# 0xb4lamx/hocuspocus

Measured on AMD Instinct MI355X. Metric: merged update MB/s (bit-exact vs yjs mergeUpdates), higher is better.
Workload: dtype u8; 1 GPU; C2: 10000 docs x 200 single-char Y.Text insert updates per GPU (documents 'c2-<i>', i < 10000, sharded by fnv1a64(name) mod 1), 1-4 uint32 clients, batched Y.mergeUpdates, inputs resident in HBM; docs_per_gpu=10000, docs_total=10000, updates_total=2000000, bytes_in_total=47221584, bytes_out_total=29357349, parallelism=doc-sharded x1

## Files before the change

hocuspocus_amd/csrc/ygm_kernels.hip:

```cpp
#include <hip/hip_runtime.h>
#include <stdint.h>
#include <stdio.h>
#include <stdlib.h>

#include <atomic>

#include "ygm_common.hpp"
#include "ygm_merge_seq.hpp"
#include "ygm_merge_wave.hpp"
#include "ygm_merge_lean.hpp"
#include "ygm_docmeta.hpp"
#include "ygm_doc_walk.hpp"
#include "ygm_merge_big.hpp"
#include "ygm_seqdoc.hpp"
#include "ygm_v1.hpp"

#ifdef YGM_DIAG
__device__ unsigned long long ygm_diag[32];
#define DIAG_T0 unsigned long long _dt = __builtin_amdgcn_s_memtime();
#define DIAG(i) do { if (threadIdx.x == 0) { unsigned long long _n = __builtin_amdgcn_s_memtime(); atomicAdd(&ygm_diag[i], _n - _dt); _dt = _n; } } while (0)
#define DIAGW(i) do { if ((threadIdx.x & 63) == 0) { unsigned long long _n = __builtin_amdgcn_s_memtime(); atomicAdd(&ygm_diag[8 + (i)], _n - _dt); _dt = _n; } } while (0)
__device__ unsigned long long ygm_diag_ts[16384 * 8];
#define DIAGL_T0 if (threadIdx.x == 0) ygm_diag_ts[(blockIdx.x & 16383u) * 8] = __builtin_amdgcn_s_memrealtime();
#define DIAGL(i) do { if (threadIdx.x == 0) ygm_diag_ts[(blockIdx.x & 16383u) * 8 + 1 + (i)] = __builtin_amdgcn_s_memrealtime(); } while (0)
// ... 815 lines not shown
        fb0 = atomicAdd(&meta->fb_count, (unsigned int)__popcll(bm));
        atomicAdd(&meta->fb_upds, (unsigned long long)su);
        atomicAdd(&meta->fb_bytes, (unsigned long long)sb);
      }
      fb0 = (uint32_t)__shfl((int)fb0, (int)lead);
    }
    if (rm) {
      const uint32_t rl = (uint32_t)__builtin_ctzll(rm);
      if (l == rl) r0 = atomicAdd(&meta->route_n, (unsigned int)__popcll(rm));
      r0 = (uint32_t)__shfl((int)r0, (int)rl);
    }
    if (big) {
      fb_list[fb0 + lanes_below(bm)] = d;
      out_off[d] = merge_slot(upd_off[u0], d); out_len[d] = 0; status[d] = ST_FALLBACK;
    } else if (in) rest[r0 + lanes_below(rm)] = d;
  }
}


struct LeanHdr { uint32_t u0, k; uint64_t b0, nbytes; };

YDEV uint32_t lean_du_load(const uint32_t* __restrict__ doc_upd, uint32_t d, uint32_t n_docs) {
  const uint32_t l = threadIdx.x;
  return d < n_docs ? doc_upd[d + (l & 1u)] : 0u;
}
template <int LENS>
YDEV uint64_t lean_bo_load(const uint64_t* __restrict__ upd_off, const uint64_t* __restrict__ doc_off, uint32_t du, uint32_t d,
                           uint32_t n_docs) {
  if (LENS) return d < n_docs ? doc_off[d + (threadIdx.x & 1u)] : 0ull;
  const uint32_t u0 = rdlane(du, 0), u1 = rdlane(du, 1);
  return d < n_docs ? upd_off[(threadIdx.x & 1u) ? u1 : u0] : 0ull;
}
YDEV LeanHdr lean_hdr_of(uint32_t du, uint64_t bo) {
  LeanHdr h;
  h.u0 = rdlane(du, 0); h.k = rdlane(du, 1) - h.u0;
  const uint64_t b0 = ((uint64_t)rdlane((uint32_t)(bo >> 32), 0) << 32) | rdlane((uint32_t)bo, 0);
  const uint64_t b1 = ((uint64_t)rdlane((uint32_t)(bo >> 32), 1) << 32) | rdlane((uint32_t)bo, 1);
  h.b0 = b0; h.nbytes = b1 - b0;
  return h;
}
YDEV bool ln_owns(uint32_t l, int q, uint32_t n) { return l < ((n + (uint32_t)(LN_ROWS - 1 - q)) >> 2); }
template <int WIDE>
YDEV bool lean_stageable(const LeanHdr& h) {
  return h.k >= 2 && h.k < (uint32_t)(WAVE * LN_ROWS) && (h.b0 & 15u) + h.nbytes <= (uint64_t)LnCfg<WIDE>::IN;
}
template <int WIDE, int LENS = 0>
YDEV void lean_prefetch(const uint8_t* __restrict__ arena, const uint64_t* __restrict__ upd_off, const uint16_t* __restrict__ upd_len,
                        const LeanHdr& h, bool go, u32x4 (&v)[(LnCfg<WIDE>::IN + 16 * WAVE - 1) / (16 * WAVE)],
                        uint32_t (&rx)[LN_ROWS + 1]) {
  const uint32_t l = threadIdx.x;
  const uint64_t a0 = go ? (h.b0 & ~15ull) : 0ull;
  const uint32_t last = go ? (uint32_t)(((h.b0 & 15u) + h.nbytes + 15) / 16) - 1u : 0u;
#pragma unroll
  for (int j = 0; j < (LnCfg<WIDE>::IN + 16 * WAVE - 1) / (16 * WAVE); j++) {
    const uint32_t c = l + WAVE * j;
    v[j] = *(const u32x4*)(arena + a0 + 16ull * (c < last ? c : last));
  }
  const uint32_t kk = go ? h.k : 0u;
  const uint32_t l4 = LN_ROWS * lane_opaque();
  if (LENS) {
#pragma unroll
    for (int q = 0; q < LN_ROWS; q++) {
      const uint32_t i = l4 + q;
      rx[q] = upd_len[h.u0 + (i < kk ? i : 0u)];
    }
    return;
  }
  const uint32_t* off32 = (const uint32_t*)upd_off;
#pragma unroll
  for (int q = 0; q <= LN_ROWS; q++) {
    const uint32_t i = l4 + q;
    rx[q] = off32[2ull * (h.u0 + (i <= kk ? i : 0u))];
  }
}

template <int WIDE, int LENS = 0>
#ifndef YGM_LN_OCC
#define YGM_LN_OCC 4
#endif
__global__ __launch_bounds__(WAVE, WIDE ? 3 : YGM_LN_OCC) void k_merge_lean(const uint8_t* __restrict__ arena, const uint64_t* __restrict__ upd_off,
                                                     const uint32_t* __restrict__ doc_upd, uint32_t n_docs, uint32_t flags,
                                                     uint8_t* __restrict__ out, uint64_t* __restrict__ out_off,
                                                     uint64_t* __restrict__ out_len, int32_t* __restrict__ status, DocMeta* meta,
                                                     DocMeta* __restrict__ meta_next, uint32_t* __restrict__ defer_list, uint64_t out_cap,
                                                     const uint32_t* __restrict__ list, uint32_t n_list,
                                                     const uint64_t* __restrict__ doc_off, const uint16_t* __restrict__ upd_len) {
  typedef LnCfg<WIDE> C;
  __shared__ LeanLdsT<WIDE> LS;
  if (meta_next && blockIdx.x == 0) {
    static_assert(sizeof(DocMeta) % 16 == 0, "DocMeta is zeroed in 16-byte pieces");
    const u32x4 z = {0u, 0u, 0u, 0u};
    for (uint32_t i = threadIdx.x; i < sizeof(DocMeta) / 16; i += WAVE) ((u32x4*)meta_next)[i] = z;
  }
  LB8* lin = (LB8*)LS.in;
  LB8* lout = (LB8*)LS.out;
  const uint32_t l = threadIdx.x;
  const uint32_t G = gridDim.x;
  const bool force_seq = (flags & 2u) != 0;
  const uint32_t n_it = WIDE ? n_list : n_docs;
  auto list_at = [&](uint32_t j) -> uint32_t {
    const uint64_t i = (uint64_t)blockIdx.x + (uint64_t)j * G;
    return i < n_it ? (list ? list[i] : (uint32_t)i) : n_docs;
  };
  uint32_t lst0 = 0, lst1 = 0;
  if (WIDE) { lst0 = list_at(l); lst1 = list_at(WAVE + l); }
  uint32_t it = 0;
  auto docof = [&](uint32_t j) -> uint32_t {
    return (uint32_t)__builtin_amdgcn_readfirstlane((int)rdlane((j >> 6) != (it >> 6) ? lst1 : lst0, j & 63u));
  };
#define LN_AHEAD(k) (WIDE ? docof(it + (k)) : d + (k) * G)
  uint32_t d = WIDE ? (n_it > blockIdx.x ? docof(0) : n_docs) : blockIdx.x;
  (void)n_it;
  uint32_t du = lean_du_load(doc_upd, d, n_docs);
  LeanHdr hn = lean_hdr_of(du, lean_bo_load<LENS>(upd_off, doc_off, du, d, n_docs));
  du = lean_du_load(doc_upd, LN_AHEAD(1), n_docs);
  u32x4 v[(C::IN + 16 * WAVE - 1) / (16 * WAVE)];
  uint32_t rx[LN_ROWS + 1];
#pragma unroll
  for (int q = 0; q <= LN_ROWS; q++) rx[q] = 0;
  bool gn = !force_seq && lean_stageable<WIDE>(hn);
  lean_prefetch<WIDE, LENS>(arena, upd_off, upd_len, hn, gn, v, rx);
  uint64_t payload = 0;
  uint64_t dmask = 0;
  uint32_t dit = 0, dch = d;
  auto flush_defer = [&]() {
    if (!dmask) return;
    uint32_t base = 0;
    if (l == 0) base = atomicAdd(WIDE ? &meta->wide_defer : &meta->lean_defer, (uint32_t)__popcll(dmask));
    base = __shfl(base, 0, WAVE);
    if ((dmask >> l) & 1ull) defer_list[base + lanes_below(dmask)] = WIDE ? lst0 : dch + l * G;
    dmask = 0;
  };
  DIAGSW_T0
  for (; WIDE ? (uint64_t)blockIdx.x + (uint64_t)it * G < n_it : d < n_docs; it++) {
    DIAGL_T0
    if (dit == 64) {
      flush_defer(); dit = 0; dch = d;
      if (WIDE) { lst0 = lst1; lst1 = list_at(it + WAVE + l); }
    }
    const LeanHdr h = hn;
    bool go = gn;
    const uint32_t k = h.k;
    const uint64_t b0 = h.b0, nbytes = h.nbytes;
    const uint64_t slot = merge_slot(b0, d), cap = merge_slot_cap(nbytes);
    const uint32_t shift = (uint32_t)(b0 & 15u);
    uint32_t us[LN_ROWS], un[LN_ROWS];
    DIAGSW_WAIT;
    if (go) {
      const uint32_t nch = (uint32_t)((shift + nbytes + 15) / 16);
#pragma unroll
      for (int j = 0; j < (C::IN + 16 * WAVE - 1) / (16 * WAVE); j++) {
        const uint32_t c = l + WAVE * j;
        if (c < nch) *(LB128*)(lin + 16 * c) = v[j];
      }
      if (LENS) {
        uint32_t tot = 0;
#pragma unroll
        for (int q = 0; q < LN_ROWS; q++) {
          un[q] = ln_owns(l, q, k) ? rx[q] : 0u;
          us[q] = tot;
          tot += un[q];
        }
        const uint32_t inc = dpp_incl_add(tot);
        const uint32_t base = shift + inc - tot;
#pragma unroll
        for (int q = 0; q < LN_ROWS; q++) us[q] += base;
        if (lane63(inc) != (uint32_t)nbytes) go = false;
      } else {
#pragma unroll
        for (int q = 0; q < LN_ROWS; q++) { us[q] = shift + (rx[q] - (uint32_t)b0); un[q] = rx[q + 1] - rx[q]; }
      }
      if (!WIDE) {
        bool lng = false;
#pragma unroll
        for (int q = 0; q < LN_ROWS; q++) lng |= ln_owns(l, q, k) && un[q] > (uint32_t)LN_UMAX;
        if (__ballot(lng)) go = false;
      }
    }
    __builtin_amdgcn_s_waitcnt(0x0F70);
    wave_sync();
    DIAGL(0);
#if defined(YGM_LEAN_STOP) && YGM_LEAN_STOP == 1
    { hn = lean_hdr_of(du, lean_bo_load<LENS>(upd_off, doc_off, du, LN_AHEAD(1), n_docs)); du = lean_du_load(doc_upd, LN_AHEAD(2), n_docs);
      gn = !force_seq && lean_stageable<WIDE>(hn); lean_prefetch<WIDE, LENS>(arena, upd_off, upd_len, hn, gn, v, rx); wave_sync(); dit++; d = LN_AHEAD(1); continue; }
#endif
    const uint64_t bo_next = lean_bo_load<LENS>(upd_off, doc_off, du, LN_AHEAD(1), n_docs);
    const uint32_t du_next = lean_du_load(doc_upd, LN_AHEAD(2), n_docs);
    const bool single = k < 2 && !force_seq;
    bool defer = !go && !single;
    uint32_t size = 0;
    if (single) {
      size = k == 0 ? 2u : (uint32_t)nbytes;
      if (k == 1 && nbytes > 0xFFFFFFFFull) size = 0;
      uint8_t* o = out + slot;
      const bool badlen = upd_len != nullptr && k == 1 && (uint64_t)upd_len[h.u0] != nbytes;
      uint64_t olen = k == 0 ? 2 : nbytes;
      int32_t ost = ST_OK;
      if (badlen) { size = 0; olen = 0; ost = ST_MALFORMED; }
      else if (slot + olen > out_cap) { size = 0; olen = 0; ost = ST_NOMEM; }
      else {
        if (k == 0) { if (l == 0) { o[0] = 0; o[1] = 0; } }
        else for (uint64_t c = lane_opaque(); c * 16 < nbytes; c += WAVE) {
          uint4 x; __builtin_memcpy(&x, arena + b0 + 16 * c, 16);
          *(uint4*)(o + 16 * c) = x;
        }
        payload += olen;
      }
      if (l == 0) { out_off[d] = slot; out_len[d] = olen; status[d] = ost; }
      __builtin_amdgcn_s_waitcnt(0x0F70);
    }
    LRec rec[LN_ROWS];
    bool hs[LN_ROWS], hasd[LN_ROWS];
    bool bad = false;
    bool allfast = false;
#pragma unroll
    for (int q = 0; q < LN_ROWS; q++) { hs[q] = false; hasd[q] = false; }
    if (go && !WIDE && YGM_LN_FASTPARSE) {
      allfast = true;
#pragma unroll
      for (int q = 0; q < LN_ROWS; q++) {
        const bool valid = ln_owns(l, q, k);
        us[q] = valid ? us[q] : shift; un[q] = valid ? un[q] : 0u;
      }
      bool slow[LN_ROWS];
#pragma unroll
      for (int g = 0; g < LN_ROWS; g += YGM_LN_FASTGROUP) {
        LFastIn F[YGM_LN_FASTGROUP];
#pragma unroll
        for (int q = g; q < g + YGM_LN_FASTGROUP; q++) lean_fast_load(lin, us[q], un[q], F[q - g]);
#pragma unroll
        for (int q = g; q < g + YGM_LN_FASTGROUP; q++) {
          const bool valid = ln_owns(l, q, k);
          bool hd;
          const bool fast = q == 0 ? lean_parse_fast<true>(F[q - g], us[q], un[q], valid, rec[q], hd)
                                   : lean_parse_fast<false>(F[q - g], us[q], un[q], valid, rec[q], hd);
          slow[q] = !fast && valid;
          hs[q] = valid && (rec[q].span & 0xFF00u) != 0u;
          hasd[q] = valid && hd;
        }
      }
#pragma unroll
      for (int q = 0; q < LN_ROWS; q++) {
        if (__ballot(slow[q]) == 0) continue;
        allfast = false;
        const bool valid = ln_owns(l, q, k);
        if (valid) { rec[q] = lean_parse<LN_UMAX>(lin, us[q], un[q]); bad |= !rec[q].ok; }
        hs[q] = valid && (rec[q].span & 0xFF00u) != 0u;
        hasd[q] = valid && rec[q].ok && lin[lean_ds_pos(us[q], rec[q].span)] != 0;
      }
    } else if (go) {
#pragma unroll
      for (int q = 0; q < LN_ROWS; q++) {
        const bool valid = ln_owns(l, q, k);
        if (valid) { rec[q] = lean_parse<WIDE ? LNW_UMAX : LN_UMAX>(lin, us[q], un[q]); bad |= !rec[q].ok; }
        else { rec[q].ok = true; rec[q].client = 0; rec[q].clock = 0; rec[q].clen = 0; rec[q].span = 0; }
        hs[q] = valid && (rec[q].span & 0xFF00u) != 0u;
        hasd[q] = valid && rec[q].ok && lin[lean_ds_pos(us[q], rec[q].span)] != 0;
      }
    }
    DIAGL(1);
#ifdef YGM_LEAN_SB
    __builtin_amdgcn_sched_barrier(0);
#endif
    hn = lean_hdr_of(du, bo_next); du = du_next;
    gn = !force_seq && lean_stageable<WIDE>(hn);
    lean_prefetch<WIDE, LENS>(arena, upd_off, upd_len, hn, gn, v, rx);
    defer = defer || __ballot(bad) != 0;
    if (single) { wave_sync(); dit++; d = LN_AHEAD(1); continue; }
#if defined(YGM_LEAN_STOP) && YGM_LEAN_STOP == 2
    if (l == 0) status[d] = (int)bad; wave_sync(); dit++; d = LN_AHEAD(1); continue;
#endif
    if (!defer) {
      uint32_t blk[LN_ROWS];
#pragma unroll
      for (int q = 0; q < LN_ROWS; q++) blk[q] = hs[q] ? 0xFFu : 0xFEu;
      uint32_t ctl = 0, nC = 0;
      uint32_t fcl = 0, fcb[LN_ROWS];
#pragma unroll
      for (int q = 0; q < LN_ROWS; q++) fcb[q] = 0;
      bool sighted = false;
      if (!WIDE && allfast) {
        uint32_t cid[4] = {0u, 0u, 0u, 0u}, fck[4] = {0u, 0u, 0u, 0u};
        bool more = true;
#pragma unroll
        for (int t = 0; t < 4; t++) {
          const bool u0 = blk[0] == 0xFFu, u1 = blk[1] == 0xFFu, u2 = blk[2] == 0xFFu, u3 = blk[3] == 0xFFu;
          const uint64_t m = __builtin_amdgcn_ballot_w64(u0 || u1 || u2 || u3);
          if (m == 0) { more = false; break; }
          const uint32_t fl = (uint32_t)__builtin_ctzll(m);
          const uint32_t cand = rdlane(u0 ? rec[0].client : u1 ? rec[1].client : u2 ? rec[2].client : rec[3].client, fl);
          const uint32_t fc = rdlane(u0 ? rec[0].clock : u1 ? rec[1].clock : u2 ? rec[2].clock : rec[3].clock, fl);
          cid[t] = cand; fck[t] = fc; nC = (uint32_t)t + 1u;
#pragma unroll
          for (int q = 0; q < LN_ROWS; q++) {
            const bool hit = blk[q] == 0xFFu && rec[q].client == cand;
            blk[q] = hit ? 8u * (uint32_t)t : blk[q];
            fcb[q] = hit ? fc : fcb[q];
          }
        }
        if (more) more = __builtin_amdgcn_ballot_w64(blk[0] == 0xFFu || blk[1] == 0xFFu || blk[2] == 0xFFu || blk[3] == 0xFFu) != 0;
        if (more) {
#pragma unroll
          for (int q = 0; q < LN_ROWS; q++) blk[q] = hs[q] ? 0xFFu : 0xFEu;
          nC = 0;
        } else {
          sighted = true;
          uint32_t tab = 0;
#pragma unroll
          for (int t = 3; t >= 0; t--) {
            uint32_t r = 0;
#pragma unroll
            for (int j = 0; j < 4; j++) if (j != t) r = lean_sadd_gt(r, cid[j], cid[t]);
            tab |= r << (8 * t);
            lean_wrlane2(ctl, cid[t], fcl, fck[t], r);
          }
#pragma unroll
          for (int q = 0; q < LN_ROWS; q++) blk[q] = __builtin_amdgcn_ubfe(tab, blk[q], 8u);
        }
      }
      for (int it = 0; !sighted && it <= LN_CMAX; it++) {
        uint32_t mx = 0; bool any = false;
#pragma unroll
        for (int q = 0; q < LN_ROWS; q++) { const bool un_ = blk[q] == 0xFFu; any |= un_; mx = max(mx, un_ ? rec[q].client : 0u); }
        if (__ballot(any) == 0) break;
        if (nC == (uint32_t)LN_CMAX) { defer = true; break; }
        const uint32_t cand = lane63(dpp_incl_max(mx));
#pragma unroll
        for (int q = 0; q < LN_ROWS; q++) if (blk[q] == 0xFFu && rec[q].client == cand) blk[q] = nC;
        ctl = l == nC ? cand : ctl;
        nC++;
      }
      if (!defer) {
        uint32_t cA = 0, cB = 0;
        uint32_t idx[LN_ROWS];
        {
          uint32_t ea[LN_ROWS], ta = 0;
#pragma unroll
          for (int q = 0; q < LN_ROWS; q++) {
            ea[q] = ta;
            ta += (hs[q] && blk[q] < 4u) ? 1u << (8u * (blk[q] & 3u)) : 0u;
          }
          const uint32_t ia = dpp_incl_add(ta);
          cA = lane63(ia);
#pragma unroll
          for (int q = 0; q < LN_ROWS; q++) idx[q] = ia - ta + ea[q];
          if (nC > 4u) {
            uint32_t eb[LN_ROWS], tb = 0;
#pragma unroll
            for (int q = 0; q < LN_ROWS; q++) {
              eb[q] = tb;
              tb += (hs[q] && blk[q] >= 4u) ? 1u << (8u * (blk[q] & 3u)) : 0u;
            }
            const uint32_t ib = dpp_incl_add(tb);
            cB = lane63(ib);
#pragma unroll
            for (int q = 0; q < LN_ROWS; q++) idx[q] = (hs[q] && blk[q] >= 4u) ? ib - tb + eb[q] : idx[q];
          }
#pragma unroll
          for (int q = 0; q < LN_ROWS; q++) idx[q] = (idx[q] >> (8u * (blk[q] & 3u))) & 0xFFu;
        }
        uint32_t osp[LN_ROWS], oex[LN_ROWS];
        uint32_t carry = 0, hcnt = 0, hfc = 0, hpos = 0, hdr_all = 0, HC0 = 0, HC1 = 0, nrec = 0;
        const bool logp = sighted;
        if (logp) {
#pragma unroll
          for (int q = 0; q < LN_ROWS; q++) bad |= hs[q] && rec[q].clock != fcb[q] + idx[q];
          const uint32_t T01 = lean_byte_prefix<0>(hs, blk, rec, osp);
          uint32_t T23 = 0;
          if (nC > 2u) T23 = lean_byte_prefix<1>(hs, blk, rec, osp);
          const uint32_t B0 = T01 & 0xFFFFu, B1 = T01 >> 16, B2 = T23 & 0xFFFFu, B3 = T23 >> 16;
          uint32_t hlen = 0;
          if (l < nC) {
            hcnt = (cA >> (8u * (l & 3u))) & 0xFFu; hfc = fcl;
            hlen = vlen32(hcnt) + vlen32(ctl) + vlen32(hfc);
          }
          const uint32_t h0 = rdlane(hlen, 0), h1 = rdlane(hlen, 1), h2 = rdlane(hlen, 2), h3 = rdlane(hlen, 3);
          const uint32_t O0 = vlen32(nC) + h0, O1 = O0 + h1 + B0, O2 = O1 + h2 + B1, O3 = O2 + h3 + B2;
          const uint32_t O01 = O0 | (O1 << 16), O23 = O2 | (O3 << 16);
          hdr_all = h0 + h1 + h2 + h3;
          carry = B0 + B1 + B2 + B3;
          hpos = lean_field16((l & 2u) ? O23 : O01, l) - hlen;
#pragma unroll
// ... 2252 lines not shown
```

hocuspocus_amd/csrc/ygm_merge_lean.hpp:

```cpp
#pragma once
#include "ygm_common.hpp"
#include "ygm_merge_wave.hpp"

namespace ygm {

#ifndef YGM_LN_IN
#define YGM_LN_IN 5120
#endif
#ifndef YGM_LN_OUT
#define YGM_LN_OUT 4096
#endif
constexpr int LN_IN = YGM_LN_IN;
constexpr int LN_ROWS = 4;
constexpr int LN_UMAX = 32;
constexpr int LN_CMAX = 8;

constexpr int LN_OUT = YGM_LN_OUT;

constexpr int LNW_IN = 7168;
constexpr int LNW_UMAX = 64;
constexpr int LNW_OUT = 6144;

template <int WIDE> struct LnCfg {
  static constexpr int IN = WIDE ? LNW_IN : LN_IN;
// ... 69 lines not shown
}

YDEV uint32_t lean_ds_pos(uint32_t us, uint32_t span) { return span ? (span >> 16) + (span & 0xFFu) : us + 1u; }

struct LRec {
  uint32_t client, clock, clen;
  uint32_t span;
  bool ok;
};

YDEV uint32_t pext32(uint32_t x, uint32_t y, uint32_t n) {
  x &= n >= 4u ? 0xFFFFFFFFu : ((1u << (8u * n)) - 1u);
  x &= 0x7f7f7f7fu;
  x = ((x >> 1) & 0x3f803f80u) | (x & 0x007f007fu);
  x = ((x >> 2) & 0x0fffc000u) | (x & 0x00003fffu);
  return x | (n >= 5u ? (y & 0x7Fu) << 28 : 0u);
}

YDEV uint32_t bsel(uint32_t m, uint32_t x, uint32_t y) { return (x & m) | (y & ~m); }

template <int W>
YDEV void lean_windowW(LB8* in, uint32_t s, uint32_t (&d)[W / 4]) {
  const LB32* w = (const LB32*)(in + (s & ~3u));
  uint32_t L[W / 4 + 1];
#pragma unroll
  for (int j = 0; j <= W / 4; j++) L[j] = w[j];
#pragma unroll
  for (int j = 0; j < W / 4; j++) d[j] = __builtin_amdgcn_alignbyte(L[j + 1], L[j], s & 3u);
}
YDEV void lean_window(LB8* in, uint32_t s, uint32_t (&d)[8]) { lean_windowW<32>(in, s, d); }
YDEV uint32_t top8(uint32_t lo, uint32_t hi) {
  const uint32_t a = __builtin_amdgcn_udot4(lo & 0x80808080u, 0x08040201u, 0u, false);
  return __builtin_amdgcn_udot4(hi & 0x80808080u, 0x80402010u, a, false) >> 7;
}
template <int W> struct LnMask;
template <> struct LnMask<32> { typedef uint32_t T; };
template <> struct LnMask<64> { typedef uint64_t T; };
template <int W>
YDEV typename LnMask<W>::T lean_hmaskW(const uint32_t (&d)[W / 4]) {
  typename LnMask<W>::T H = 0;
#pragma unroll
  for (int j = 0; j < W / 8; j++) H |= (typename LnMask<W>::T)top8(d[2 * j], d[2 * j + 1]) << (8 * j);
  return H;
}
YDEV uint32_t lean_hmask(const uint32_t (&d)[8]) { return lean_hmaskW<32>(d); }
YDEV uint32_t lnctz(uint32_t x) { return (uint32_t)__builtin_ctz(x | 0x80000000u); }
YDEV uint32_t lnctz(uint64_t x) { return (uint32_t)__builtin_ctzll(x | 0x8000000000000000ull); }

template <int W>
YDEV LRec lean_parse(LB8* in, uint32_t s, uint32_t n) {
  typedef typename LnMask<W>::T M;
  constexpr uint32_t WB = (uint32_t)W, WL = WB - 1u;
  constexpr M ONE = 1, ALL = ~(M)0;
  LRec R; R.ok = false; R.client = 0; R.clock = 0; R.clen = 0; R.span = 0;
  if (n < 2 || n > WB) return R;
  uint32_t d[W / 4];
  lean_windowW<W>(in, s, d);
  if ((d[0] & 0xFFu) == 0u) { R.ok = true; return R; }
  const M H = lean_hmaskW<W>(d);
  M Z = 0;
#pragma unroll
  for (int j = 0; j < W / 8; j++)
    Z |= (M)top8((d[2 * j] - 0x01010101u) & ~d[2 * j], (d[2 * j + 1] - 0x01010101u) & ~d[2 * j + 1]) << (8 * j);
  const M V = n >= WB ? ALL : ((ONE << n) - ONE);
  const M T = ~H & V;
  const M HV = H & V;
  LB8* u = in + s;
  const M h2 = HV & (HV >> 1), h4 = h2 & (h2 >> 2), h7 = h4 & (h4 >> 3);
  M bad = h7 | (Z & (HV << 1) & V);
#define LN_VEND(p, e) ((e) = ((p) < WL ? (p) : WL) + lnctz((M)(T >> ((p) < WL ? (p) : WL))))
#define LN_ASCII(p, L) (bad |= (M)(((n - (p) - (L)) & 0x80000000u) | ((L) & ~WL)) | ((HV >> ((p) < WL ? (p) : WL)) & ((ONE << ((L) & WL)) - ONE)))
  const uint32_t b0 = d[0] & 0xFFu, b1 = (d[0] >> 8) & 0xFFu;
  bad |= (M)((b0 ^ 1u) | ((b1 - 1u) & ~127u) | (n < 4u ? 1u : 0u));
  uint32_t e, p;
  LN_VEND(2u, e);
  const uint32_t cl_n = e - 1u;
  const uint32_t client = pext32(__builtin_amdgcn_alignbyte(d[1], d[0], 2u), (d[1] >> 16) & 0xFFu, cl_n);
  bad |= (M)((cl_n > 5u ? 1u : 0u) | (cl_n == 5u ? ((d[1] >> 16) & 0x70u) : 0u));
  p = e + 1u;
  LN_VEND(p, e);
  const uint32_t ck_n = e - p + 1u;
  const uint64_t U01 = ((uint64_t)d[1] << 32) | d[0], U23 = ((uint64_t)d[3] << 32) | d[2];
  const uint64_t cw = (U01 >> (8u * (p & 7u))) | (p & 7u ? (U23 << (64u - 8u * (p & 7u))) : 0ull);
  const uint32_t clock = pext32((uint32_t)cw, (uint32_t)(cw >> 32) & 0xFFu, ck_n);
  bad |= (M)((ck_n > 5u ? 1u : 0u) | (ck_n == 5u ? ((uint32_t)(cw >> 32) & 0x70u) : 0u));
  p = e + 1u;
  const uint32_t sstart = p;
  uint32_t clen = 0;
  constexpr uint32_t PC = WB + 8u;
  uint32_t st = 0;
  do {
    const uint32_t pc = p < PC ? p : PC;
    const uint32_t info = u[pc];
    p = pc + 1u;
    const uint32_t ref = info & 31u;
    bad |= (M)((info == 10u ? 1u : 0u) | ((ref != 1u && ref != 4u) ? 1u : 0u) | ((info & 0xC0u) && (info & 0x20u) ? 1u : 0u));
    {
      const uint32_t pp = p < WL ? p : WL;
      const M t0 = (T >> pp) | (ONE << WL), t1 = t0 & (t0 - ONE), t2 = t1 & (t1 - ONE), t3 = t2 & (t2 - ONE);
      const uint32_t nsk = ((info >> 6) & 1u) + ((info >> 7) & 1u);
      const uint32_t e2 = pp + lnctz(t1) + 1u;
      const uint32_t e4 = pp + lnctz(t3) + 1u;
      p = nsk == 2u ? e4 : nsk == 1u ? e2 : p;
    }
    if ((info & 0xC0u) == 0u) {
      const uint32_t pi = u[p < PC ? p : PC]; p++;
      if (pi == 1u) {
        const uint32_t Lk = u[p < PC ? p : PC]; p++;
        LN_ASCII(p, Lk); p += Lk & WL;
      } else {
        bad |= (M)pi;
        LN_VEND(p, e); p = e + 1u; LN_VEND(p, e); p = e + 1u;
      }
      if (info & 0x20u) {
        const uint32_t Ls = u[p < PC ? p : PC]; p++;
        LN_ASCII(p, Ls); p += Ls & WL;
      }
    }
    if (ref == 1u) {
      LN_VEND(p, e);
      const uint32_t pp = p < WL ? p : WL;
      const uint32_t x = u[pp] | ((uint32_t)u[pp + 1] << 8) | ((uint32_t)u[pp + 2] << 16) | ((uint32_t)u[pp + 3] << 24);
      const uint32_t v = pext32(x, 0u, e - p + 1u);
      bad |= (M)((v == 0u ? 1u : 0u) | ((e - p) > 2u ? 1u : 0u));
      clen += v;
      p = e + 1u;
    } else {
      const uint32_t Lc = u[p < PC ? p : PC]; p++;
      bad |= (M)(Lc == 0u ? 1u : 0u);
      LN_ASCII(p, Lc);
      p += Lc & WL;
      clen += Lc;
    }
  } while (++st < b1 && (bad | (M)(p >= n ? 1u : 0u)) == 0);
#undef LN_VEND
#undef LN_ASCII
  bad |= (M)((n - 1u - p) & 0x80000000u);
  bad |= (M)(uint32_t)(((uint64_t)clock + clen) >> 32);
  R.ok = bad == 0;
  R.client = client; R.clock = clock; R.clen = clen;
  R.span = ((s + sstart) << 16) | (b1 << 8) | ((p - sstart) & 0xFFu);
  return R;
}

#ifndef YGM_LN_FASTPARSE
#define YGM_LN_FASTPARSE 1
#endif
#ifndef YGM_LN_FASTGROUP
#define YGM_LN_FASTGROUP 4
#endif
#ifndef YGM_LN_FASTPARENT
#define YGM_LN_FASTPARENT 1
#endif
struct LFastIn {
  uint32_t d[8];
  uint32_t tl, td;
};
YDEV void lean_fast_load(LB8* in, uint32_t s, uint32_t n, LFastIn& F) {
  lean_window(in, s, F.d);
  const uint32_t t = s + (n > 3u ? n : 3u);
  F.tl = in[t - 3u]; F.td = in[t - 1u];
}
#ifndef YGM_LN_KEYGATE
#define YGM_LN_KEYGATE 1
#endif
template <bool KEYROW>
YDEV bool lean_parse_fast(const LFastIn& F, uint32_t s, uint32_t n, bool valid, LRec& R, bool& hasd) {
  const uint32_t (&d)[8] = F.d;
  const uint32_t H = lean_hmask(d);
  uint32_t Z = 0;
#pragma unroll
  for (int j = 0; j < 4; j++)
    Z |= top8((d[2 * j] - 0x01010101u) & ~d[2 * j], (d[2 * j + 1] - 0x01010101u) & ~d[2 * j + 1]) << (8 * j);
  const uint32_t V = n >= 32u ? 0xFFFFFFFFu : ((1u << n) - 1u);
  const uint32_t T = ~H & V, HV = H & V;
  const uint32_t h2 = HV & (HV >> 1), h4 = h2 & (h2 >> 2), h7 = h4 & (h4 >> 3);
  uint32_t bad = h7 | (Z & (HV << 1) & V);
  const uint32_t b0 = d[0] & 0xFFu, b1 = (d[0] >> 8) & 0xFFu;
  bad |= (b0 ^ 1u) | (b1 ^ 1u);
  uint32_t e = 2u + lnctz(T >> 2);
  const uint32_t cl_n = e - 1u;
  const uint32_t client = pext32(__builtin_amdgcn_alignbyte(d[1], d[0], 2u), (d[1] >> 16) & 0xFFu, cl_n);
  bad |= (cl_n > 5u ? 1u : 0u) | (cl_n == 5u ? ((d[1] >> 16) & 0x70u) : 0u);
  const uint32_t p = e + 1u;
  const uint32_t pc = p < 31u ? p : 31u;
  e = pc + lnctz(T >> pc);
  const uint32_t ck_n = e - p + 1u;
  const uint64_t U01 = ((uint64_t)d[1] << 32) | d[0], U23 = ((uint64_t)d[3] << 32) | d[2];
  const uint64_t cw = (U01 >> (8u * (p & 7u))) | (p & 7u ? (U23 << (64u - 8u * (p & 7u))) : 0ull);
  const uint32_t clock = pext32((uint32_t)cw, (uint32_t)(cw >> 32) & 0xFFu, ck_n);
  bad |= (ck_n > 5u ? 1u : 0u) | (ck_n == 5u ? ((uint32_t)(cw >> 32) & 0x70u) : 0u);
  bad |= clock == 0xFFFFFFFFu ? 1u : 0u;
  const uint32_t ip = e + 1u;
  const uint32_t x3 = (uint32_t)(cw >> (8u * (ck_n & 7u)));
  const uint32_t info = x3 & 0xFFu;
  const uint32_t nsk = ((info >> 6) & 1u) + ((info >> 7) & 1u);
  const uint32_t pp = ip + 1u < 31u ? ip + 1u : 31u;
  const uint32_t t0 = (T >> pp) | 0x80000000u, t1 = t0 & (t0 - 1u), t2 = t1 & (t1 - 1u), t3 = t2 & (t2 - 1u);
  const uint32_t pl = nsk == 2u ? pp + lnctz(t3) + 1u : pp + lnctz(t1) + 1u;
  bool fits = pl + 3u == n;
  bool shape = nsk != 0u && (info & 0x3Fu) == 4u;
#if YGM_LN_FASTPARENT
  if (KEYROW || !YGM_LN_KEYGATE || __ballot(valid && nsk == 0u) != 0) {
    const uint32_t lk = (x3 >> 16) & 0xFFu;
    const uint32_t kp = ip + 3u < 31u ? ip + 3u : 31u;
    const bool par = x3 << 16 == 0x01040000u && lk < 32u && ((HV >> kp) & ((1u << (lk & 31u)) - 1u)) == 0u;
    fits = nsk == 0u ? ip + 6u + lk == n : fits;
    shape = shape || (nsk == 0u && par);
  }
#endif
  const bool item = bad == 0u && shape && fits && n <= 32u && F.tl == 1u && ((HV >> ((n - 2u) & 31u)) & 1u) == 0u;
  const bool dsonly = b0 == 0u && n >= 2u && n <= 32u;
  R.ok = true;
  R.client = item ? client : 0u; R.clock = item ? clock : 0u; R.clen = item ? 1u : 0u;
  R.span = item ? ((s + ip) << 16) | (1u << 8) | ((n - 1u - ip) & 0xFFu) : 0u;
  hasd = item ? F.td != 0u : b1 != 0u;
  return item || dsonly;
}

YDEV uint32_t w2_byte(const uint32_t (&d)[8], uint32_t p) {
  const uint32_t i = p >> 2;
  const uint32_t m0 = 0u - (i & 1u), m1 = 0u - ((i >> 1) & 1u), m2 = 0u - ((i >> 2) & 1u);
  const uint32_t a0 = bsel(m0, d[1], d[0]), a1 = bsel(m0, d[3], d[2]), a2 = bsel(m0, d[5], d[4]), a3 = bsel(m0, d[7], d[6]);
  const uint32_t b0 = bsel(m1, a1, a0), b1 = bsel(m1, a3, a2);
  return (bsel(m2, b1, b0) >> (8u * (p & 3u))) & 0xFFu;
}
YDEV void w2_vu5(const uint32_t (&d)[8], uint32_t p, uint32_t& x, uint32_t& y) {
  const uint32_t i = p >> 2, s = p & 3u;
  const uint32_t m0 = 0u - (i & 1u), m1 = 0u - ((i >> 1) & 1u);
  const uint32_t lo = bsel(m1, bsel(m0, d[3], d[2]), bsel(m0, d[1], d[0]));
  const uint32_t hi = bsel(m1, bsel(m0, d[4], d[3]), bsel(m0, d[2], d[1]));
  const uint32_t hh = bsel(m1, bsel(m0, d[5], d[4]), bsel(m0, d[3], d[2]));
  x = __builtin_amdgcn_alignbyte(hi, lo, s);
  y = __builtin_amdgcn_alignbyte(hh, hi, s) & 0xFFu;
}

constexpr int LN_DSMAX = 64;
struct LDsCur {
  LB8* u;
  uint32_t T, lim;
  uint32_t p, cl_left, r_left, client, bad;
};
YDEV uint32_t lean_ds_vu(LDsCur& c, uint32_t maxb) {
  const uint32_t pp = c.p < 31u ? c.p : 31u;
  const uint32_t e = pp + (uint32_t)__builtin_ctz((c.T >> pp) | 0x80000000u);
  const uint32_t nb = e - c.p + 1u;
  LB8* b = c.u + pp;
  const uint32_t x = b[0] | ((uint32_t)b[1] << 8) | ((uint32_t)b[2] << 16) | ((uint32_t)b[3] << 24), y = b[4];
  c.bad |= (c.p >= c.lim ? 1u : 0u) | (e >= c.lim ? 1u : 0u) | (nb > maxb ? 1u : 0u) | (nb == 5u ? (y & 0x70u) : 0u);
  c.p = e + 1u;
  return pext32(x, y, nb);
}
YDEV void lean_ds_open(LB8* in, uint32_t a, uint32_t n, LDsCur& c) {
  uint32_t d[8];
  lean_window(in, a, d);
  c.u = in + a;
  c.lim = n < 32u ? n : 32u;
  c.T = ~lean_hmask(d) & (c.lim >= 32u ? 0xFFFFFFFFu : ((1u << c.lim) - 1u));
  c.p = 0; c.bad = 0; c.r_left = 0; c.client = 0;
  c.cl_left = lean_ds_vu(c, 4u);
}
YDEV bool lean_ds_more(const LDsCur& c) { return c.bad == 0u && (c.r_left | c.cl_left) != 0u; }
YDEV void lean_ds_next(LDsCur& c, uint32_t& client, uint32_t& clock, uint32_t& len) {
  if (c.r_left == 0u) {
    c.client = lean_ds_vu(c, 5u);
    c.r_left = lean_ds_vu(c, 4u);
    c.bad |= c.r_left == 0u ? 1u : 0u;
    c.cl_left--;
  }
  client = c.client;
  clock = lean_ds_vu(c, 4u);
  len = lean_ds_vu(c, 4u);
  c.r_left -= c.r_left ? 1u : 0u;
}

template <int ND>
YDEV void lds_or_copy(LB8* out, LB8* in, uint32_t t, uint32_t s, uint32_t n) {
  const uint32_t head = t & 3u;
  const uint32_t src0 = s - head;
  const uint32_t sb = src0 & 3u;
  LB32* sw = (LB32*)(in + (src0 & ~3u));
  uint32_t w[ND + 1];
#pragma unroll
  for (int j = 0; j <= ND; j++) w[j] = sw[j];
  LB32* od = (LB32*)(out + (t & ~3u));
  const uint32_t last = head + n;
  const uint32_t jl = (last - 1u) >> 2;
  const uint32_t mtail = 0xFFFFFFFFu >> (8u * (4u * jl + 4u - last));
#pragma unroll
  for (int j = 0; j < ND; j++) {
    const uint32_t v = __builtin_amdgcn_alignbyte(w[j + 1], w[j], sb);
    uint32_t m = (uint32_t)j < jl ? 0xFFFFFFFFu : (uint32_t)j == jl ? mtail : 0u;
    if (j == 0) m &= 0xFFFFFFFFu << (8u * head);
    __hip_atomic_fetch_or(od + j, v & m, __ATOMIC_RELAXED, __HIP_MEMORY_SCOPE_WORKGROUP);
  }
}
template <int WIDE>
YDEV uint32_t lean_copy_class(uint32_t cw) {
  if (__ballot(cw > 24u) == 0) return 0u;
  return (!WIDE || __ballot(cw > 36u) == 0) ? 1u : 2u;
}
template <int WIDE>
YDEV void lean_copy(LB8* out, LB8* in, uint32_t cls, bool go, uint32_t t, uint32_t s, uint32_t n) {
  if (!go) return;
  if (cls == 0u) lds_or_copy<6>(out, in, t, s, n);
  else if (!WIDE || cls == 1u) lds_or_copy<9>(out, in, t, s, n);
  else lds_or_copy<17>(out, in, t, s, n);
}
YDEV uint32_t lds_vu(LB8* out, uint32_t t, uint32_t v) {
  while (v > 127u) { out[t++] = (uint8_t)(0x80u | (v & 127u)); v >>= 7; }
  out[t++] = (uint8_t)v;
  return t;
}

YDEV uint32_t vlen32(uint32_t v) {
  return 1u + (v > 0x7Fu ? 1u : 0u) + (v > 0x3FFFu ? 1u : 0u) + (v > 0x1FFFFFu ? 1u : 0u) + (v > 0xFFFFFFFu ? 1u : 0u);
}
YDEV uint32_t lean_sadd_gt(uint32_t r, uint32_t a, uint32_t b) {
  asm("s_cmp_gt_u32 %1, %2\n\ts_addc_u32 %0, %0, 0" : "+s"(r) : "s"(a), "s"(b) : "scc");
  return r;
}
YDEV void lean_wrlane2(uint32_t& x, uint32_t vx, uint32_t& y, uint32_t vy, uint32_t lane) {
  uint32_t keep;
  asm("s_mov_b32 %2, m0\n\ts_mov_b32 m0, %5\n\ts_nop 0\n\tv_writelane_b32 %0, %3, m0\n\tv_writelane_b32 %1, %4, m0\n\ts_mov_b32 m0, %2"
      : "+v"(x), "+v"(y), "=&s"(keep) : "s"(vx), "s"(vy), "s"(lane));
}
YDEV uint32_t lean_field16(uint32_t x, uint32_t b) { return (x >> (16u * (b & 1u))) & 0xFFFFu; }
template <int HI>
YDEV uint32_t lean_byte_prefix(const bool (&hs)[LN_ROWS], const uint32_t (&blk)[LN_ROWS], const LRec (&rec)[LN_ROWS],
                               uint32_t (&pre)[LN_ROWS]) {
  uint32_t e[LN_ROWS], t = 0;
  bool in[LN_ROWS];
#pragma unroll
  for (int q = 0; q < LN_ROWS; q++) {
    in[q] = hs[q] && (blk[q] >> 1) == (uint32_t)HI;
    e[q] = t;
    t += in[q] ? (rec[q].span & 0xFFu) << (16u * (blk[q] & 1u)) : 0u;
  }
  const uint32_t inc = dpp_incl_add(t);
#pragma unroll
  for (int q = 0; q < LN_ROWS; q++) pre[q] = (HI == 0 || in[q]) ? inc - t + e[q] : pre[q];
  return lane63(inc);
}

template <int CTRL, int RM, bool BC>
YDEV void dpp_max64_step(uint32_t& hi, uint32_t& lo) {
  const uint32_t h2 = (uint32_t)__builtin_amdgcn_update_dpp(0, (int)hi, CTRL, RM, 0xF, BC);
  const uint32_t l2 = (uint32_t)__builtin_amdgcn_update_dpp(0, (int)lo, CTRL, RM, 0xF, BC);
  const bool gt = h2 > hi || (h2 == hi && l2 > lo);
  hi = gt ? h2 : hi; lo = gt ? l2 : lo;
}
template <int J>
YDEV uint32_t lane_xor(uint32_t x, uint32_t l) {
  if (J == 1) return (uint32_t)__builtin_amdgcn_update_dpp(0, (int)x, 0xB1, 0xF, 0xF, false);
  if (J == 2) return (uint32_t)__builtin_amdgcn_update_dpp(0, (int)x, 0x4E, 0xF, 0xF, false);
  if (J == 4 || J == 8) {
    const uint32_t up = (uint32_t)__builtin_amdgcn_update_dpp(0, (int)x, 0x100 | J, 0xF, 0xF, false);
    const uint32_t dn = (uint32_t)__builtin_amdgcn_update_dpp(0, (int)x, 0x110 | J, 0xF, 0xF, false);
    return (l & J) ? dn : up;
  }
  return (uint32_t)__shfl_xor((int)x, J, 64);
}
template <int K, int J>
YDEV void bitonic_step(uint32_t& a, uint32_t& b, uint32_t& c, uint32_t l) {
  const uint32_t oa = lane_xor<J>(a, l), ob = lane_xor<J>(b, l), oc = lane_xor<J>(c, l);
  const bool lt = oa < a || (oa == a && (ob < b || (ob == b && oc < c)));
  const bool lower = (l & J) == 0, asc = (l & K) == 0;
  const bool take = lower == asc ? lt : !lt;
  a = take ? oa : a; b = take ? ob : b; c = take ? oc : c;
}
template <int K, int J>
YDEV void bitonic_merge(uint32_t& a, uint32_t& b, uint32_t& c, uint32_t l) {
  bitonic_step<K, J>(a, b, c, l);
  if constexpr (J > 1) bitonic_merge<K, J / 2>(a, b, c, l);
}
YDEV void lane_bitonic3(uint32_t& a, uint32_t& b, uint32_t& c) {
  const uint32_t l = lane_opaque();
  bitonic_merge<2, 1>(a, b, c, l);
  bitonic_merge<4, 2>(a, b, c, l);
  bitonic_merge<8, 4>(a, b, c, l);
  bitonic_merge<16, 8>(a, b, c, l);
  bitonic_merge<32, 16>(a, b, c, l);
  bitonic_merge<64, 32>(a, b, c, l);
}
YDEV uint64_t lean_max_scan64(uint64_t v) {
  uint32_t hi = (uint32_t)(v >> 32), lo = (uint32_t)v;
  dpp_max64_step<0x111, 0xF, true>(hi, lo);
  dpp_max64_step<0x112, 0xF, true>(hi, lo);
  dpp_max64_step<0x114, 0xF, true>(hi, lo);
  dpp_max64_step<0x118, 0xF, true>(hi, lo);
  dpp_max64_step<0x142, 0xA, false>(hi, lo);
  dpp_max64_step<0x143, 0xC, false>(hi, lo);
  return ((uint64_t)hi << 32) | lo;
}

struct LDsUnion {
  uint32_t client, nruns, sclock, rend;
  bool segstart, runend;
  uint32_t pos;
  uint32_t nsegs, bytes;
  bool bad;
};
#ifdef YGM_DIAG
static __device__ unsigned long long ygm_diag_ds[4];
#define LDS_T0 unsigned long long _dst = __builtin_amdgcn_s_memtime();
#define LDS_STAMP(i) do { const unsigned long long _n = __builtin_amdgcn_s_memtime(); if (threadIdx.x == 0) atomicAdd(&ygm_diag_ds[i], _n - _dst); _dst = _n; } while (0)
#else
#define LDS_T0
#define LDS_STAMP(i)
#endif
YDEV LDsUnion lean_ds_union(LB8* lin, LB32* scr, const uint32_t (&dpos)[LN_ROWS], const uint32_t (&uend)[LN_ROWS],
                            const bool (&hasd)[LN_ROWS], uint32_t flags) {
  const uint32_t l = threadIdx.x;
  LDsUnion U; U.bad = false; U.nsegs = 0; U.bytes = 1; U.segstart = false; U.runend = false; U.pos = 0;
  U.client = 0; U.nruns = 0; U.sclock = 0; U.rend = 0;
  LB32* rc = scr; LB32* rk = scr + LN_DSMAX; LB32* re = scr + 2 * LN_DSMAX;
  LB32* rn = scr + 3 * LN_DSMAX;
  uint32_t nrec = 0, bad = 0;
  LDS_T0
#pragma unroll
  for (int q = 0; q < LN_ROWS; q++) {
    if (__ballot(hasd[q]) == 0) continue;
    bool fq = false;
    uint32_t fcl = 0, fck = 0, fln = 0;
    if (hasd[q]) {
      uint32_t w[8];
      lean_window(lin, dpos[q], w);
      const uint32_t n = uend[q] - dpos[q], lim = n < 32u ? n : 32u;
      const uint32_t T = ~lean_hmask(w) & (lim >= 32u ? 0xFFFFFFFFu : ((1u << lim) - 1u));
      const uint32_t t1 = T & (T - 1u), t2 = t1 & (t1 - 1u), t3 = t2 & (t2 - 1u), t4 = t3 & (t3 - 1u);
      const uint32_t e1 = lnctz(T), e2 = lnctz(t1), e3 = lnctz(t2), e4 = lnctz(t3), e5 = lnctz(t4);
      uint32_t cx, cy, kx, ky, lx, ly;
      w2_vu5(w, 1u, cx, cy);
      w2_vu5(w, (e3 + 1u) & 15u, kx, ky);
      w2_vu5(w, (e4 + 1u) & 15u, lx, ly);
      const uint32_t ncb = e2 - e1, nkb = e4 - e3, nlb = e5 - e4;
      fq = e1 == 0u && (w[0] & 0xFFu) == 1u && e3 == e2 + 1u && w2_byte(w, e3 & 31u) == 1u && e5 < lim &&
           ncb - 1u <= 4u && !(ncb == 5u && (cy & 0x70u)) && nkb - 1u <= 3u && nlb - 1u <= 3u;
      fcl = pext32(cx, cy, ncb); fck = pext32(kx, ky, nkb); fln = pext32(lx, ly, nlb);
    }
    {
      const uint64_t m = __ballot(fq);
      const uint32_t slot = nrec + lanes_below(m);
      if (fq && slot < (uint32_t)LN_DSMAX) { rc[slot] = fcl; rk[slot] = fck; re[slot] = fck + fln; rn[slot] = ((uint32_t)LN_ROWS * lane_opaque() + q) << 8; }
      nrec += (uint32_t)__builtin_popcountll(m);
    }
    const bool slow = hasd[q] && !fq;
    if (__ballot(slow) == 0) continue;
    LDsCur c;
    if (slow) lean_ds_open(lin, dpos[q], uend[q] - dpos[q], c);
    else { c.bad = 0; c.cl_left = 0; c.r_left = 0; }
    for (int it = 0; it < LN_DSMAX; it++) {
      bool has = lean_ds_more(c);
      if (__ballot(has) == 0) break;
      uint32_t cl = 0, ck = 0, ln = 0;
      if (has) lean_ds_next(c, cl, ck, ln);
      has = has && c.bad == 0u;
      const uint64_t m = __ballot(has);
// ... 67 lines not shown
```

Measured before the change: 2.135 million MB/s.

## Precompute per-chunk high-bit and zero-byte masks in LDS during input staging

While staging each 16-byte input chunk into LDS, the lean path now computes the high-bit and zero-byte bitmasks with udot4 and writes them as 16-bit entries into the (not yet used) output buffer. The fast parser reads a 32-bit window of each mask with alignbit instead of loading 32 bytes and deriving the masks per row, so the byte window it loads shrinks to 16. A narrower copy variant (5 dwords) is also added for waves whose copy widths all fit in 20 bytes. This trades extra ALU work and LDS writes during staging for less per-row LDS traffic and mask arithmetic. It relies on the output buffer not being written before parsing finishes.

```diff
diff --git a/hocuspocus_amd/csrc/ygm_kernels.hip b/hocuspocus_amd/csrc/ygm_kernels.hip
--- a/hocuspocus_amd/csrc/ygm_kernels.hip
+++ b/hocuspocus_amd/csrc/ygm_kernels.hip
@@ -991,6 +991,11 @@
       for (int j = 0; j < (C::IN + 16 * WAVE - 1) / (16 * WAVE); j++) {
         const uint32_t c = l + WAVE * j;
         if (c < nch) *(LB128*)(lin + 16 * c) = v[j];
+        if (!WIDE) {
+          uint32_t mh, mz;
+          lean_chunk_masks(v[j], mh, mz);
+          if (c < nch) { ((LB16*)lout)[c] = (uint16_t)mh; ((LB16*)(lout + LN_MASKB))[c] = (uint16_t)mz; }
+        }
       }
       if (LENS) {
         uint32_t tot = 0;
@@ -1066,7 +1071,7 @@
       for (int g = 0; g < LN_ROWS; g += YGM_LN_FASTGROUP) {
         LFastIn F[YGM_LN_FASTGROUP];
 #pragma unroll
-        for (int q = g; q < g + YGM_LN_FASTGROUP; q++) lean_fast_load(lin, us[q], un[q], F[q - g]);
+        for (int q = g; q < g + YGM_LN_FASTGROUP; q++) lean_fast_load(lin, lout, us[q], un[q], F[q - g]);
 #pragma unroll
         for (int q = g; q < g + YGM_LN_FASTGROUP; q++) {
           const bool valid = ln_owns(l, q, k);
diff --git a/hocuspocus_amd/csrc/ygm_merge_lean.hpp b/hocuspocus_amd/csrc/ygm_merge_lean.hpp
--- a/hocuspocus_amd/csrc/ygm_merge_lean.hpp
+++ b/hocuspocus_amd/csrc/ygm_merge_lean.hpp
@@ -245,12 +245,29 @@
 #ifndef YGM_LN_FASTPARENT
 #define YGM_LN_FASTPARENT 1
 #endif
+constexpr int LN_MASKB = LN_IN / 8 + 8;
+static_assert(LN_MASKB % 4 == 0 && 2 * LN_MASKB <= LN_OUT, "two bit arrays of whole dwords in the output buffer");
+typedef __attribute__((address_space(3))) uint16_t LB16;
+YDEV void lean_chunk_masks(const u32x4& v, uint32_t& h, uint32_t& z) {
+  constexpr uint32_t M = 0x80808080u, W0 = 0x08040201u, W1 = 0x80402010u, ONES = 0x01010101u;
+  const uint32_t ha = __builtin_amdgcn_udot4(v[1] & M, W1, __builtin_amdgcn_udot4(v[0] & M, W0, 0u, false), false);
+  const uint32_t hb = __builtin_amdgcn_udot4(v[3] & M, W1, __builtin_amdgcn_udot4(v[2] & M, W0, 0u, false), false);
+  h = (ha >> 7) | (hb << 1);
+  const uint32_t za = __builtin_amdgcn_udot4((v[1] - ONES) & ~v[1] & M, W1, __builtin_amdgcn_udot4((v[0] - ONES) & ~v[0] & M, W0, 0u, false), false);
+  const uint32_t zb = __builtin_amdgcn_udot4((v[3] - ONES) & ~v[3] & M, W1, __builtin_amdgcn_udot4((v[2] - ONES) & ~v[2] & M, W0, 0u, false), false);
+  z = (za >> 7) | (zb << 1);
+}
 struct LFastIn {
-  uint32_t d[8];
+  uint32_t d[4];
+  uint32_t H, Z;
   uint32_t tl, td;
 };
-YDEV void lean_fast_load(LB8* in, uint32_t s, uint32_t n, LFastIn& F) {
-  lean_window(in, s, F.d);
+YDEV void lean_fast_load(LB8* in, LB8* masks, uint32_t s, uint32_t n, LFastIn& F) {
+  lean_windowW<16>(in, s, F.d);
+  const LB32* mh = (const LB32*)masks + (s >> 5);
+  const LB32* mz = mh + LN_MASKB / 4;
+  F.H = __builtin_amdgcn_alignbit(mh[1], mh[0], s & 31u);
+  F.Z = __builtin_amdgcn_alignbit(mz[1], mz[0], s & 31u);
   const uint32_t t = s + (n > 3u ? n : 3u);
   F.tl = in[t - 3u]; F.td = in[t - 1u];
 }
@@ -259,12 +276,8 @@
 #endif
 template <bool KEYROW>
 YDEV bool lean_parse_fast(const LFastIn& F, uint32_t s, uint32_t n, bool valid, LRec& R, bool& hasd) {
-  const uint32_t (&d)[8] = F.d;
-  const uint32_t H = lean_hmask(d);
-  uint32_t Z = 0;
-#pragma unroll
-  for (int j = 0; j < 4; j++)
-    Z |= top8((d[2 * j] - 0x01010101u) & ~d[2 * j], (d[2 * j + 1] - 0x01010101u) & ~d[2 * j + 1]) << (8 * j);
+  const uint32_t (&d)[4] = F.d;
+  const uint32_t H = F.H, Z = F.Z;
   const uint32_t V = n >= 32u ? 0xFFFFFFFFu : ((1u << n) - 1u);
   const uint32_t T = ~H & V, HV = H & V;
   const uint32_t h2 = HV & (HV >> 1), h4 = h2 & (h2 >> 2), h7 = h4 & (h4 >> 3);
@@ -388,15 +401,20 @@
     __hip_atomic_fetch_or(od + j, v & m, __ATOMIC_RELAXED, __HIP_MEMORY_SCOPE_WORKGROUP);
   }
 }
+#ifndef YGM_LN_COPY5
+#define YGM_LN_COPY5 1
+#endif
 template <int WIDE>
 YDEV uint32_t lean_copy_class(uint32_t cw) {
+  if (!WIDE && YGM_LN_COPY5 && __ballot(cw > 20u) == 0) return 3u;
   if (__ballot(cw > 24u) == 0) return 0u;
   return (!WIDE || __ballot(cw > 36u) == 0) ? 1u : 2u;
 }
 template <int WIDE>
 YDEV void lean_copy(LB8* out, LB8* in, uint32_t cls, bool go, uint32_t t, uint32_t s, uint32_t n) {
   if (!go) return;
-  if (cls == 0u) lds_or_copy<6>(out, in, t, s, n);
+  if (!WIDE && YGM_LN_COPY5 && cls == 3u) lds_or_copy<5>(out, in, t, s, n);
+  else if (cls == 0u) lds_or_copy<6>(out, in, t, s, n);
   else if (!WIDE || cls == 1u) lds_or_copy<9>(out, in, t, s, n);
   else lds_or_copy<17>(out, in, t, s, n);
 }
```

Measured after the change: 2.292 million MB/s (median of 6 runs). +7.4%, better.
